# zhangxinsong-nlp/XFM

Hardware: AMD Instinct MI355X
Metric: image-text pairs/sec fwd+bwd, XFM-base 224px/30tok (higher is better)
Workload: dtype bf16; 1 GPU; Pretrain.py full multimodal step (ITC+ITM+MLM+MIM), XFM-base, synthetic 224px images + 30-token captions, random init; units_per_gpu=64, global_batch=64, dropout=True, ordered_reductions=True, grad_allreduce=False, parallelism=dp1, image_res=224

## Files before the change

### xfm_amd/csrc/gemm.hip

```cpp
#include "common.h"

enum { EPI_BF16 = 0, EPI_F32 = 1, EPI_GELU = 2, EPI_DGELU = 3, EPI_F32_ACC = 4 };

#define XFM_FENCE() asm volatile("" ::: "memory")
#define XFM_BAR()                    \
  do {                               \
    XFM_FENCE();                     \
    __builtin_amdgcn_s_barrier();    \
    XFM_FENCE();                     \
  } while (0)


struct GemmNT {
  const bf16* A; long lda;
  const bf16* B; long ldb;
  void* C; long ldc;
  const float* bias;
  bf16* aux; long ldaux;
  int M, N, K;
  int group_m;
  int k_splits;
  long split_stride;
#ifdef XFM_DIAG
  long long* dbg;
// ... 810 lines not shown

__device__ __forceinline__ int swz_t(int r) { return ((r & 3) | (((r >> 3) & 1) << 2)) << 1; }

__device__ __forceinline__ bf16x8 tr_read_pair(const char* tile, int row0, int col0, int lr) {
  const int r = row0 + (lr >> 2);
  const int col = col0 + 4 * (lr & 3);
  const int off0 = r * 256 + ((((col >> 3)) ^ swz_t(r)) << 4) + (col & 7) * 2;
  const int r2 = r + 4;
  const int off1 = r2 * 256 + ((((col >> 3)) ^ swz_t(r2)) << 4) + (col & 7) * 2;
  const s16x4 lo = __builtin_amdgcn_ds_read_tr16_b64_v4i16(LDS_PTR(s16x4, tile + off0));
  const s16x4 hi = __builtin_amdgcn_ds_read_tr16_b64_v4i16(LDS_PTR(s16x4, tile + off1));
  union { struct { s16x4 a, b; } s; bf16x8 v; } u;
  u.s.a = lo;
  u.s.b = hi;
  return u.v;
}

__global__ __launch_bounds__(256) void gemm_tn_kernel(GemmTN g) {
  constexpr int TILE = 64 * 256;
  extern __shared__ __attribute__((aligned(16))) char smem[];
  const int tid = threadIdx.x, lane = tid & 63, w = tid >> 6;
  const int wn = w >> 1, wk = w & 1;
  const int lr = lane & 15, lg = lane >> 4;
  const int tiles_k = (g.K + 127) / 128, tiles_n = (g.N + 127) / 128;
  const int per_split = tiles_k * tiles_n;
  const int wg = xcd_remap(blockIdx.x, gridDim.x);
  const int split = wg / per_split, t = wg % per_split;
  const int n0 = (t / tiles_k) * 128, k0 = (t % tiles_k) * 128;
  const int mbeg = split * g.m_per_split;
  int mend = mbeg + g.m_per_split;
  mend = mend < g.M ? mend : g.M;
  const int nsteps = (mend - mbeg + 63) / 64;

  const bool do_bias = g.dbias != nullptr && k0 == 0;
  float bsum[8] = {0.f, 0.f, 0.f, 0.f, 0.f, 0.f, 0.f, 0.f};
  u32x4 ry[4], rx[4];
  auto gload = [&](int step) {
    const int mb = mbeg + step * 64;
#pragma unroll
    for (int i = 0; i < 4; ++i) {
      const int q = i * 256 + tid, r = q >> 4, c = q & 15;
      const int m = mb + r;
      const bool okm = m < mend;
      const int nn = n0 + c * 8, kk = k0 + c * 8;
      ry[i] = u32x4{0, 0, 0, 0};
      rx[i] = u32x4{0, 0, 0, 0};
      if (okm && nn < g.N) {
        if (nn + 8 <= g.N) ry[i] = *reinterpret_cast<const u32x4*>(g.dY + (long)m * g.ldy + nn);
        else {
          union { bf16 h[8]; u32x4 v; } u; u.v = u32x4{0, 0, 0, 0};
          for (int e = 0; e < 8; ++e) if (nn + e < g.N) u.h[e] = g.dY[(long)m * g.ldy + nn + e];
          ry[i] = u.v;
        }
      }
      if (okm && kk < g.K) rx[i] = *reinterpret_cast<const u32x4*>(g.X + (long)m * g.ldx + kk);
    }
  };
  auto lstore = [&](int buf) {
    char* sY = smem + buf * 2 * TILE;
    char* sX = sY + TILE;
#pragma unroll
    for (int i = 0; i < 4; ++i) {
      const int q = i * 256 + tid, r = q >> 4, c = q & 15;
      const int off = r * 256 + ((c ^ swz_t(r)) << 4);
      *reinterpret_cast<u32x4*>(sY + off) = ry[i];
      *reinterpret_cast<u32x4*>(sX + off) = rx[i];
      if (do_bias) {
#pragma unroll
        for (int e = 0; e < 4; ++e) {
          bsum[2 * e] += __uint_as_float(ry[i][e] << 16);
          bsum[2 * e + 1] += __uint_as_float(ry[i][e] & 0xFFFF0000u);
        }
      }
    }
  };

  f32x4 acc[4][4];
#pragma unroll
  for (int i = 0; i < 4; ++i)
#pragma unroll
    for (int j = 0; j < 4; ++j) acc[i][j] = f32x4{0.f, 0.f, 0.f, 0.f};

  if (nsteps > 0) {
    gload(0);
    lstore(0);
  }
  __syncthreads();
  for (int s = 0; s < nsteps; ++s) {
    const int cur = s & 1;
    if (s + 1 < nsteps) gload(s + 1);
    const char* sY = smem + cur * 2 * TILE;
    const char* sX = sY + TILE;
#pragma unroll
    for (int ks = 0; ks < 2; ++ks) {
      bf16x8 af[4], bfr[4];
#pragma unroll
      for (int nt = 0; nt < 4; ++nt) af[nt] = tr_read_pair(sY, ks * 32 + 8 * lg, wn * 64 + nt * 16, lr);
#pragma unroll
      for (int kt = 0; kt < 4; ++kt) bfr[kt] = tr_read_pair(sX, ks * 32 + 8 * lg, wk * 64 + kt * 16, lr);
#pragma unroll
      for (int nt = 0; nt < 4; ++nt)
#pragma unroll
        for (int kt = 0; kt < 4; ++kt)
          acc[nt][kt] = __builtin_amdgcn_mfma_f32_16x16x32_bf16(af[nt], bfr[kt], acc[nt][kt], 0, 0, 0);
    }
    if (s + 1 < nsteps) lstore(cur ^ 1);
    __syncthreads();
  }

  if (do_bias) {
    float* red = reinterpret_cast<float*>(smem);
    __syncthreads();
#pragma unroll
    for (int e = 0; e < 8; ++e) red[(tid >> 4) * 128 + (tid & 15) * 8 + e] = bsum[e];
    __syncthreads();
    if (tid < 128 && n0 + tid < g.N) {
      float t2 = 0.f;
#pragma unroll
      for (int r = 0; r < 16; ++r) t2 += red[r * 128 + tid];
      atomicAdd(g.dbias + n0 + tid, t2);
    }
  }
  if (g.ws != nullptr) {
    f32x4* wsp = reinterpret_cast<f32x4*>(g.ws) + ((((long)split * per_split + t) * 4 + w) * 16) * 64 + lane;
#pragma unroll
    for (int nt = 0; nt < 4; ++nt)
#pragma unroll
      for (int kt = 0; kt < 4; ++kt) wsp[(nt * 4 + kt) * 64] = acc[nt][kt];
    return;
  }
#pragma unroll
  for (int nt = 0; nt < 4; ++nt)
#pragma unroll
    for (int kt = 0; kt < 4; ++kt) {
      const int k = k0 + wk * 64 + kt * 16 + lr;
#pragma unroll
      for (int rgi = 0; rgi < 4; ++rgi) {
        const int n = n0 + wn * 64 + nt * 16 + 4 * lg + rgi;
        if (n < g.N && k < g.K) {
          float* dst = g.dW + (long)n * g.ldw + k;
          if (g.direct) *dst += acc[nt][kt][rgi];
          else atomicAdd(dst, acc[nt][kt][rgi]);
        }
      }
    }
}


__device__ __attribute__((aligned(256))) static const uint32_t g_zero_row[64] = {0};

__global__ __launch_bounds__(256) void gemm_tn_ring_kernel(GemmTN g, TnBatch bt) {
  constexpr int IMG = 32 * 256, STG = 2 * IMG, NS = 4;
  extern __shared__ __attribute__((aligned(16))) char smem[];
  const int tid = threadIdx.x, lane = tid & 63, w = tid >> 6;
  const int wn = w >> 1, wk = w & 1;
  const int lr = lane & 15, lg = lane >> 4;
  const int tiles_k = g.K / 128, tiles_n = g.N / 128;
  const int per_split = tiles_k * tiles_n;
  int wg = xcd_remap(blockIdx.x, gridDim.x);
  if (bt.nb > 1) {
    const int bi = wg / bt.wg_per;
    wg -= bi * bt.wg_per;
    g.dY = bt.dY[bi];
    g.X = bt.X[bi];
    g.dW = bt.dW[bi];
    g.dbias = bt.dbias[bi];
    g.ws += (long)bi * bt.ws_stride;
  }
  const int split = wg / per_split, t = wg % per_split;
  const int n0 = (t / tiles_k) * 128, k0 = (t % tiles_k) * 128;
  const int mbeg = split * g.m_per_split;
  int mend = mbeg + g.m_per_split;
  mend = mend < g.M ? mend : g.M;
  const int nsteps = (mend - mbeg + 31) / 32;
  const bool do_bias = g.dbias != nullptr && k0 == 0 && wk == 0;

  const bf16* zrow = reinterpret_cast<const bf16*>(g_zero_row);
  int lrow[2], lcol[2];
#pragma unroll
  for (int i = 0; i < 2; ++i) {
    lrow[i] = 4 * (i * 4 + w) + (lane >> 4);
    lcol[i] = ((lane & 15) ^ swz_t(lrow[i])) * 8;
  }
  auto issue = [&](int s) {
    if (s >= nsteps) return;
    char* base = smem + (s & (NS - 1)) * STG;
#pragma unroll
    for (int i = 0; i < 2; ++i) {
      const int m = mbeg + s * 32 + lrow[i];
      const bool ok = m < mend;
      const bf16* sy = ok ? g.dY + (long)m * g.ldy + n0 + lcol[i] : zrow + lcol[i];
      const bf16* sx = ok ? g.X + (long)m * g.ldx + k0 + lcol[i] : zrow + lcol[i];
      const unsigned dy_lds = (unsigned)(uintptr_t)LDS_PTR(void, base) + (unsigned)__builtin_amdgcn_readfirstlane((i * 4 + w) * 1024);
      asm volatile("s_mov_b32 m0, %1\n\ts_nop 0\n\tglobal_load_lds_dwordx4 %0, off" ::"v"(sy), "s"(dy_lds) : "memory", "m0");
      asm volatile("s_mov_b32 m0, %1\n\ts_nop 0\n\tglobal_load_lds_dwordx4 %0, off" ::"v"(sx), "s"(dy_lds + (unsigned)IMG) : "memory", "m0");
    }
  };

  f32x4 acc[4][4];
#pragma unroll
  for (int i = 0; i < 4; ++i)
#pragma unroll
    for (int j = 0; j < 4; ++j) acc[i][j] = f32x4{0.f, 0.f, 0.f, 0.f};
  f32x4 bacc[4];
#pragma unroll
  for (int i = 0; i < 4; ++i) bacc[i] = f32x4{0.f, 0.f, 0.f, 0.f};
  bf16x8 ones;
#pragma unroll
  for (int i = 0; i < 8; ++i) ones[i] = f2bf(1.0f);

  issue(0);
  issue(1);
  issue(2);
  for (int s = 0; s < nsteps; ++s) {
    const int younger = nsteps - 1 - s < 2 ? nsteps - 1 - s : 2;
    if (younger == 2) asm volatile("s_waitcnt vmcnt(8)" ::: "memory");
    else if (younger == 1) asm volatile("s_waitcnt vmcnt(4)" ::: "memory");
    else asm volatile("s_waitcnt vmcnt(0)" ::: "memory");
    XFM_BAR();
    issue(s + 3);
    const char* sY = smem + (s & (NS - 1)) * STG;
    const char* sX = sY + IMG;
    bf16x8 af[4], bfr[4];
#pragma unroll
    for (int nt = 0; nt < 4; ++nt) af[nt] = tr_read_pair(sY, 8 * lg, wn * 64 + nt * 16, lr);
#pragma unroll
    for (int kt = 0; kt < 4; ++kt) bfr[kt] = tr_read_pair(sX, 8 * lg, wk * 64 + kt * 16, lr);
#pragma unroll
    for (int nt = 0; nt < 4; ++nt)
#pragma unroll
      for (int kt = 0; kt < 4; ++kt)
        acc[nt][kt] = __builtin_amdgcn_mfma_f32_16x16x32_bf16(af[nt], bfr[kt], acc[nt][kt], 0, 0, 0);
    if (do_bias) {
#pragma unroll
      for (int nt = 0; nt < 4; ++nt) bacc[nt] = __builtin_amdgcn_mfma_f32_16x16x32_bf16(af[nt], ones, bacc[nt], 0, 0, 0);
    }
  }

  if (do_bias && lr == 0) {
#pragma unroll
    for (int nt = 0; nt < 4; ++nt)
#pragma unroll
      for (int i = 0; i < 4; ++i) atomicAdd(g.dbias + n0 + wn * 64 + nt * 16 + 4 * lg + i, bacc[nt][i]);
  }
  if (g.ws != nullptr) {
    f32x4* wsp = reinterpret_cast<f32x4*>(g.ws) + ((((long)split * per_split + t) * 4 + w) * 16) * 64 + lane;
#pragma unroll
    for (int nt = 0; nt < 4; ++nt)
#pragma unroll
      for (int kt = 0; kt < 4; ++kt) wsp[(nt * 4 + kt) * 64] = acc[nt][kt];
    return;
  }
#pragma unroll
  for (int nt = 0; nt < 4; ++nt)
#pragma unroll
    for (int kt = 0; kt < 4; ++kt) {
      const int k = k0 + wk * 64 + kt * 16 + lr;
#pragma unroll
      for (int rgi = 0; rgi < 4; ++rgi) {
        const int n = n0 + wn * 64 + nt * 16 + 4 * lg + rgi;
        float* dst = g.dW + (long)n * g.ldw + k;
        if (g.direct) *dst += acc[nt][kt][rgi];
        else atomicAdd(dst, acc[nt][kt][rgi]);
      }
    }
}

__global__ __launch_bounds__(256) void tn_reduce128_kernel(const float* __restrict__ ws, float* __restrict__ dW, long ldw, int N, int K,
                                                           int tiles_k, int per_split, int splits, TnBatch bt) {
  if (bt.nb > 1) {
    ws += (long)blockIdx.y * bt.ws_stride;
    dW = bt.dW[blockIdx.y];
  }
  const long idx = (long)blockIdx.x * 256 + threadIdx.x;
  const int lane = (int)(idx & 63), q = (int)((idx >> 6) & 15), w = (int)((idx >> 10) & 3);
  const int t = (int)(idx >> 12);
  if (t >= per_split) return;
  const f32x4* p = reinterpret_cast<const f32x4*>(ws) + idx;
  const long stride = (long)per_split * 4 * 16 * 64;
  f32x4 sum = p[0];
  for (int sp = 1; sp < splits; ++sp) sum += p[sp * stride];
  const int n0 = (t / tiles_k) * 128, k0 = (t % tiles_k) * 128;
  const int wn = w >> 1, wk = w & 1, lr = lane & 15, lg = lane >> 4, nt = q >> 2, kt = q & 3;
  const int k = k0 + wk * 64 + kt * 16 + lr;
  const int n = n0 + wn * 64 + nt * 16 + 4 * lg;
  if (k >= K) return;
#pragma unroll
  for (int i = 0; i < 4; ++i)
    if (n + i < N) dW[(long)(n + i) * ldw + k] += sum[i];
}

struct Tn256Seg {
  const bf16* dY; const bf16* X;
  unsigned ldy, ldx;
  int n0, k0, mbeg, nk;
  bool do_bias;
  int rows;
};
__device__ __attribute__((aligned(16))) const unsigned tn_zero16[4] = {0u, 0u, 0u, 0u};

template <bool RAGGED>
__device__ __forceinline__ void tn256_mainloop(const Tn256Seg& sg, char* smem, f32x4 (&acc)[8][4], f32x4 (&bacc)[2]) {
  constexpr int UNIT = 64 * 256, BUF = 4 * UNIT;
  const int tid = threadIdx.x, lane = tid & 63, w = tid >> 6;
  const int wr = w >> 2, wc = w & 3;
  const int lr = lane & 15, lg = lane >> 4;
  const int n0 = sg.n0, k0 = sg.k0, mbeg = sg.mbeg, nk = sg.nk;
  const int total = 4 * nk;
  const bool do_bias = sg.do_bias;

  unsigned soff[4][2];
  int doff[4][2];
#pragma unroll
  for (int i = 0; i < 2; ++i) {
    const int b = i * 8 + w;
    const int r = 4 * b + (lane >> 4);
    const int c = ((lane & 15) ^ swz_t(r)) * 8;
    const unsigned rowy = (unsigned)(mbeg + r) * (unsigned)sg.ldy, rowx = (unsigned)(mbeg + r) * (unsigned)sg.ldx;
    soff[0][i] = rowy + n0 + (c >> 6) * 128 + (c & 63);
    soff[3][i] = rowy + n0 + (c >> 6) * 128 + 64 + (c & 63);
    soff[1][i] = rowx + k0 + (c >> 5) * 64 + (c & 31);
    soff[2][i] = rowx + k0 + (c >> 5) * 64 + 32 + (c & 31);
    doff[0][i] = 0 * UNIT + b * 1024;
    doff[1][i] = 1 * UNIT + b * 1024;
    doff[2][i] = 2 * UNIT + b * 1024;
    doff[3][i] = 3 * UNIT + b * 1024;
  }
  auto issue = [&](int s) {
    if (s >= total) return;
    const int kt = s >> 2, j = s & 3;
    char* base = smem + (kt & 1) * BUF;
    const bool isy = (j == 0 || j == 3);
    const bf16* src = (isy ? sg.dY : sg.X) + (size_t)kt * 64 * (size_t)(isy ? sg.ldy : sg.ldx);
#pragma unroll
    for (int i = 0; i < 2; ++i) {
      const unsigned so = j == 0 ? soff[0][i] : j == 1 ? soff[1][i] : j == 2 ? soff[2][i] : soff[3][i];
      const int dofs = j == 0 ? doff[0][i] : j == 1 ? doff[1][i] : j == 2 ? doff[2][i] : doff[3][i];
      const unsigned lds_addr = (unsigned)(uintptr_t)LDS_PTR(void, base) + (unsigned)__builtin_amdgcn_readfirstlane(dofs);
      const bf16* ptr = src + (size_t)so;
      if (RAGGED && kt * 64 + 4 * (i * 8 + w) + (lane >> 4) >= sg.rows) ptr = reinterpret_cast<const bf16*>(tn_zero16);
      asm volatile("s_mov_b32 m0, %1\n\ts_nop 0\n\tglobal_load_lds_dwordx4 %0, off" ::"v"(ptr), "s"(lds_addr) : "memory", "m0");
    }
  };

#pragma unroll
  for (int i = 0; i < 8; ++i)
#pragma unroll
    for (int j = 0; j < 4; ++j) acc[i][j] = f32x4{0.f, 0.f, 0.f, 0.f};
  bacc[0] = bacc[1] = f32x4{0.f, 0.f, 0.f, 0.f};
  bf16x8 ones;
#pragma unroll
  for (int i = 0; i < 8; ++i) ones[i] = f2bf(1.0f);

  const int lrow = 8 * lg + (lr >> 2);
  const int tsw = swz_t(lrow);
  int offa[4], offb[2];
#pragma unroll
  for (int f = 0; f < 4; ++f) {
    const int col = wr * 64 + f * 16 + 4 * (lr & 3);
    offa[f] = lrow * 256 + (((col >> 3) ^ tsw) << 4) + (col & 7) * 2;
  }
#pragma unroll
  for (int f = 0; f < 2; ++f) {
    const int col = wc * 32 + f * 16 + 4 * (lr & 3);
    offb[f] = lrow * 256 + (((col >> 3) ^ tsw) << 4) + (col & 7) * 2;
  }
  auto tr_pair = [&](const char* p) {
    const s16x4 lo = __builtin_amdgcn_ds_read_tr16_b64_v4i16(LDS_PTR(s16x4, p));
    const s16x4 hi = __builtin_amdgcn_ds_read_tr16_b64_v4i16(LDS_PTR(s16x4, p + 1024));
    union { struct { s16x4 a, b; } s; bf16x8 v; } u;
    u.s.a = lo;
    u.s.b = hi;
    return u.v;
  };
  bf16x8 xa[4][2], wb0[2][2], wb1[2][2];
  auto read_a = [&](const char* unit) {
#pragma unroll
    for (int f = 0; f < 4; ++f) {
      xa[f][0] = tr_pair(unit + offa[f]);
      xa[f][1] = tr_pair(unit + offa[f] + 8192);
    }
  };
  auto read_b = [&](const char* unit, bf16x8 (&wb)[2][2]) {
#pragma unroll
    for (int f = 0; f < 2; ++f) {
      wb[f][0] = tr_pair(unit + offb[f]);
      wb[f][1] = tr_pair(unit + offb[f] + 8192);
    }
  };
#define XFM_TQUAD(MH, NH, WB)                                                                                    \
  do {                                                                                                           \
    __builtin_amdgcn_s_setprio(1);                                                                               \
    _Pragma("unroll") for (int ks = 0; ks < 2; ++ks)                                                             \
    _Pragma("unroll") for (int m = 0; m < 4; ++m)                                                                \
    _Pragma("unroll") for (int n = 0; n < 2; ++n)                                                                \
      acc[MH * 4 + m][NH * 2 + n] =                                                                              \
          __builtin_amdgcn_mfma_f32_16x16x32_bf16(xa[m][ks], WB[n][ks], acc[MH * 4 + m][NH * 2 + n], 0, 0, 0);  \
    __builtin_amdgcn_s_setprio(0);                                                                               \
  } while (0)
#define XFM_TBIAS(H)                                                                                             \
  do {                                                                                                           \
    if (do_bias) {                                                                                               \
      _Pragma("unroll") for (int f = 0; f < 4; ++f)                                                              \
        if (f == wc) {                                                                                           \
          bacc[H] = __builtin_amdgcn_mfma_f32_16x16x32_bf16(xa[f][0], ones, bacc[H], 0, 0, 0);                  \
          bacc[H] = __builtin_amdgcn_mfma_f32_16x16x32_bf16(xa[f][1], ones, bacc[H], 0, 0, 0);                  \
        }                                                                                                        \
    }                                                                                                            \
  } while (0)

#pragma unroll
  for (int s = 0; s < 5; ++s) issue(s);
  wait_younger((total - 1 < 4 ? total - 1 : 4) - 1);
  XFM_BAR();
  if (wr == 1) XFM_BAR();

  for (int kt = 0; kt < nk; ++kt) {
    const char* buf = smem + (kt & 1) * BUF;
    const int ph = 4 * kt;
    int last;
    issue(ph + 5);
    read_a(buf + 0 * UNIT);
    read_b(buf + 1 * UNIT, wb0);
    last = ph + 5 < total ? ph + 5 : total - 1;
    wait_younger(last - (ph + 2));
    XFM_BAR();
    XFM_TQUAD(0, 0, wb0);
    XFM_TBIAS(0);
    XFM_BAR();
    issue(ph + 6);
    read_b(buf + 2 * UNIT, wb1);
    last = ph + 6 < total ? ph + 6 : total - 1;
    wait_younger(last - (ph + 3));
    XFM_BAR();
    XFM_TQUAD(0, 1, wb1);
    XFM_BAR();
    issue(ph + 7);
    read_a(buf + 3 * UNIT);
    XFM_BAR();
    XFM_TQUAD(1, 1, wb1);
    XFM_TBIAS(1);
    XFM_BAR();
    issue(ph + 8);
    last = ph + 8 < total ? ph + 8 : total - 1;
    wait_younger(last - (ph + 5) < 0 ? 0 : last - (ph + 5));
    XFM_BAR();
    XFM_TQUAD(1, 0, wb0);
    XFM_BAR();
  }
  if (wr == 0) XFM_BAR();
#undef XFM_TQUAD
#undef XFM_TBIAS

}

template <bool ATOMIC>
__device__ __forceinline__ void tn256_bias_out(float* dbias, int n0, const f32x4 (&bacc)[2]) {
  const int lane = threadIdx.x & 63, w = threadIdx.x >> 6, wr = w >> 2, wc = w & 3, lr = lane & 15, lg = lane >> 4;
  if (lr != 0) return;
#pragma unroll
  for (int h = 0; h < 2; ++h)
#pragma unroll
    for (int i = 0; i < 4; ++i) {
      float* d = dbias + n0 + wr * 128 + h * 64 + wc * 16 + 4 * lg + i;
      if (ATOMIC) atomicAdd(d, bacc[h][i]);
      else *d += bacc[h][i];
    }
}
__device__ __forceinline__ void tn256_bias_part(float* part, const f32x4 (&bacc)[2]) {
  const int lane = threadIdx.x & 63, w = threadIdx.x >> 6, wr = w >> 2, wc = w & 3, lr = lane & 15, lg = lane >> 4;
  if (lr != 0) return;
#pragma unroll
  for (int h = 0; h < 2; ++h) *reinterpret_cast<f32x4*>(part + wr * 128 + h * 64 + wc * 16 + 4 * lg) = bacc[h];
}
__device__ __forceinline__ void tn256_store_partial(float* ws, long slot, const f32x4 (&acc)[8][4]) {
  const int lane = threadIdx.x & 63, w = threadIdx.x >> 6;
  f32x4* wsp = reinterpret_cast<f32x4*>(ws) + ((slot * 8 + w) * 32) * 64 + lane;
#pragma unroll
  for (int nt = 0; nt < 8; ++nt)
#pragma unroll
    for (int kt = 0; kt < 4; ++kt) wsp[(nt * 4 + kt) * 64] = acc[nt][kt];
}
template <bool ATOMIC>
__device__ __forceinline__ void tn256_add_out(float* dW, long ldw, int n0, int k0, const f32x4 (&acc)[8][4]) {
  const int lane = threadIdx.x & 63, w = threadIdx.x >> 6, wr = w >> 2, wc = w & 3, lr = lane & 15, lg = lane >> 4;
#pragma unroll
  for (int nt = 0; nt < 8; ++nt)
#pragma unroll
    for (int kt = 0; kt < 4; ++kt) {
      const int k = k0 + wc * 64 + kt * 16 + lr;
#pragma unroll
      for (int rgi = 0; rgi < 4; ++rgi) {
        const int n = n0 + wr * 128 + nt * 16 + 4 * lg + rgi;
        if (ATOMIC) atomicAdd(dW + (long)n * ldw + k, acc[nt][kt][rgi]);
        else dW[(long)n * ldw + k] += acc[nt][kt][rgi];
      }
    }
}

__global__ __launch_bounds__(512) void gemm_tn_256_kernel(GemmTN g) {
  extern __shared__ __attribute__((aligned(16))) char smem[];
  const int tiles_k = g.K / 256, tiles_n = g.N / 256;
  const int per_split = tiles_k * tiles_n;
  const int wg = xcd_remap(blockIdx.x, gridDim.x);
  const int split = wg / per_split, t = wg % per_split;
  const int n0 = (t / tiles_k) * 256, k0 = (t % tiles_k) * 256;
  const int mbeg = split * g.m_per_split;
  int mend = mbeg + g.m_per_split;
  mend = mend < g.M ? mend : g.M;
  const Tn256Seg sg{g.dY, g.X, (unsigned)g.ldy, (unsigned)g.ldx, n0, k0, mbeg, (mend - mbeg) / 64, g.dbias != nullptr && k0 == 0, 0};
  f32x4 acc[8][4], bacc[2];
  tn256_mainloop<false>(sg, smem, acc, bacc);
  if (sg.do_bias) tn256_bias_out<true>(g.dbias, n0, bacc);
  if (g.ws != nullptr) {
    tn256_store_partial(g.ws, (long)split * per_split + t, acc);
    return;
  }
  tn256_add_out<true>(g.dW, g.ldw, n0, k0, acc);
}

#define TN_GROUP_MAX 48
struct TnGroupProb {
  const bf16* dY; const bf16* X;
  float* dW; float* dbias;
  unsigned ldy, ldx;
  long ldw;
  int tiles_k;
  int tile_end;
};
struct TnGroup {
  int nprob, nk;
  int M;
  int total_tiles, full_tiles;
  int sk_wgs;
  long sk_iters;
  float* ws;
  float* ws_bias;
  TnGroupProb p[TN_GROUP_MAX];
};
__host__ __device__ __forceinline__ long tn_sk_bound(long R, int nk, int sk_wgs, int i) {
  long raw = (long)i * R / sk_wgs;
  const int rem = (int)(raw % nk);
  if (rem < 4) raw -= rem;
  else if (nk - rem < 4) raw += nk - rem;
  return raw;
}

__global__ __launch_bounds__(512) void gemm_tn_group_kernel(TnGroup G) {
  extern __shared__ __attribute__((aligned(16))) char smem[];
  const int wg = xcd_remap(blockIdx.x, gridDim.x), nwg = gridDim.x;
  int dp_t = wg;
  long sk_pos = 0, sk_end = 0;
  if (wg < G.sk_wgs) {
    sk_pos = tn_sk_bound(G.sk_iters, G.nk, G.sk_wgs, wg);
    sk_end = tn_sk_bound(G.sk_iters, G.nk, G.sk_wgs, wg + 1);
  }
  const long sk_a = sk_pos;
  bool first = true;
  for (;;) {
    int tile, it0, it1;
    long slot = -1;
    if (dp_t < G.full_tiles) {
      tile = dp_t;
      dp_t += nwg;
      it0 = 0;
      it1 = G.nk;
    } else if (sk_pos < sk_end) {
      const int rt = (int)(sk_pos / G.nk);
      const long t_end = (long)(rt + 1) * G.nk;
      it0 = (int)(sk_pos - (long)rt * G.nk);
      it1 = (int)((sk_end < t_end ? sk_end : t_end) - (long)rt * G.nk);
      tile = G.full_tiles + rt;
      if (it0 != 0 || it1 != G.nk) slot = 2l * wg + (sk_pos == sk_a ? 0 : 1);
      sk_pos = (long)rt * G.nk + it1;
    } else {
      break;
    }
    if (!first) __syncthreads();
    first = false;
    int pi = 0;
    while (pi + 1 < G.nprob && tile >= G.p[pi].tile_end) ++pi;
    const TnGroupProb& P = G.p[pi];
    const int tl = tile - (pi > 0 ? G.p[pi - 1].tile_end : 0);
    const int n0 = (tl / P.tiles_k) * 256, k0 = (tl % P.tiles_k) * 256;
    const Tn256Seg sg{P.dY, P.X, P.ldy, P.ldx, n0, k0, it0 * 64, it1 - it0, P.dbias != nullptr && k0 == 0, G.M - it0 * 64};
    f32x4 acc[8][4], bacc[2];
    tn256_mainloop<true>(sg, smem, acc, bacc);
    if (slot >= 0) {
      if (sg.do_bias) tn256_bias_part(G.ws_bias + slot * 256, bacc);
      tn256_store_partial(G.ws, slot, acc);
    } else {
      if (sg.do_bias) tn256_bias_out<false>(P.dbias, n0, bacc);
      tn256_add_out<false>(P.dW, P.ldw, n0, k0, acc);
    }
  }
}

__global__ __launch_bounds__(256) void tn_group_fixup_kernel(TnGroup G) {
  const int rt = blockIdx.y;
  const int idx = blockIdx.x * 256 + threadIdx.x;
  const long R = G.sk_iters;
  const long a = (long)rt * G.nk, b = a + G.nk;
  int i0 = (int)(a * G.sk_wgs / R);
  i0 = i0 < G.sk_wgs - 1 ? i0 : G.sk_wgs - 1;
  while (i0 > 0 && tn_sk_bound(R, G.nk, G.sk_wgs, i0) > a) --i0;
  while (i0 + 1 < G.sk_wgs && tn_sk_bound(R, G.nk, G.sk_wgs, i0 + 1) <= a) ++i0;
  int i1 = i0;
  while (i1 + 1 < G.sk_wgs && tn_sk_bound(R, G.nk, G.sk_wgs, i1 + 1) < b) ++i1;
  if (i0 == i1) return;
  const f32x4* ws = reinterpret_cast<const f32x4*>(G.ws);
  f32x4 sum = f32x4{0.f, 0.f, 0.f, 0.f};
  for (int i = i0; i <= i1; ++i) {
    const long slot = 2l * i + (tn_sk_bound(R, G.nk, G.sk_wgs, i) >= a ? 0 : 1);
    sum += ws[slot * (8 * 32 * 64) + idx];
  }
  const int tile = G.full_tiles + rt;
  int pi = 0;
  while (pi + 1 < G.nprob && tile >= G.p[pi].tile_end) ++pi;
  const TnGroupProb& P = G.p[pi];
  const int tl = tile - (pi > 0 ? G.p[pi - 1].tile_end : 0);
  const int n0 = (tl / P.tiles_k) * 256, k0 = (tl % P.tiles_k) * 256;
  const int lane = idx & 63, q = (idx >> 6) & 31, w = idx >> 11;
  const int wr = w >> 2, wc = w & 3, lr = lane & 15, lg = lane >> 4, nt = q >> 2, kt = q & 3;
  const int k = k0 + wc * 64 + kt * 16 + lr;
  const int n = n0 + wr * 128 + nt * 16 + 4 * lg;
#pragma unroll
  for (int i = 0; i < 4; ++i) P.dW[(long)(n + i) * P.ldw + k] += sum[i];
  if (blockIdx.x == 0 && P.dbias != nullptr && k0 == 0) {
    float b = 0.f;
    for (int i = i0; i <= i1; ++i) {
      const long slot = 2l * i + (tn_sk_bound(R, G.nk, G.sk_wgs, i) >= a ? 0 : 1);
      b += G.ws_bias[slot * 256 + threadIdx.x];
    }
    P.dbias[n0 + threadIdx.x] += b;
  }
}

__global__ __launch_bounds__(256) void tn_reduce_kernel(const float* __restrict__ ws, float* __restrict__ dW, long ldw, int tiles_k,
                                                        int per_split, int splits) {
  const long idx = (long)blockIdx.x * 256 + threadIdx.x;
  const int lane = (int)(idx & 63), q = (int)((idx >> 6) & 31), w = (int)((idx >> 11) & 7);
  const int t = (int)(idx >> 14);
  if (t >= per_split) return;
  const f32x4* p = reinterpret_cast<const f32x4*>(ws) + idx;
  const long stride = (long)per_split * 8 * 32 * 64;
  f32x4 sum = p[0];
  for (int sp = 1; sp < splits; ++sp) {
    const f32x4 v = p[sp * stride];
    sum += v;
  }
  const int n0 = (t / tiles_k) * 256, k0 = (t % tiles_k) * 256;
  const int wr = w >> 2, wc = w & 3, lr = lane & 15, lg = lane >> 4, nt = q >> 2, kt = q & 3;
  const int k = k0 + wc * 64 + kt * 16 + lr;
  const int n = n0 + wr * 128 + nt * 16 + 4 * lg;
#pragma unroll
  for (int i = 0; i < 4; ++i) dW[(long)(n + i) * ldw + k] += sum[i];
}

static int tn256_plan(int M, int N, int K, int& splits, int& mps) {
  const int t256 = (N / 256) * (K / 256);
  splits = 256 / t256;
  const int steps = M / 64;
  if (splits > steps / 8) splits = steps / 8;
  if (splits < 1) splits = 1;
  mps = cdiv(steps, splits) * 64;
  splits = cdiv(M, mps);
  return t256;
}

static bool tn256_eligible(long ldy, long ldx, int M, int N, int K) {
  return M % 64 == 0 && N % 256 == 0 && K % 256 == 0 && N >= 256 && K >= 256 &&
         (unsigned long)M * (unsigned long)(ldy > ldx ? ldy : ldx) < (1ul << 32);
}

#define TN_WS_MIN_BYTES (16l << 20)

static int tn128_plan(int M, int N, int K, int splits_hint, int& splits, int& mps) {
  const int tiles = cdiv(N, 128) * cdiv(K, 128);
  splits = splits_hint < 0 ? 0 : splits_hint;
  if (splits <= 0) {
    splits = (432 + tiles / 2) / tiles;
    int max_splits = M / 480;
    if (max_splits < 2 && M >= 640) max_splits = 2;
    if (splits > max_splits) splits = max_splits;
    if (splits < 1) splits = 1;
  }
  mps = cdiv(cdiv(M, splits), 64) * 64;
  splits = cdiv(M, mps);
  return tiles;
}

static int tn256_body_rows(int M, int N, int K) {
  const int M0 = M - M % 64;
  static const int min_rows = xfm_env_int("XFM_TN256_RAGGED_MIN", 8192);
  if (M % 64 == 0 || M0 < min_rows || N % 256 != 0 || K % 256 != 0) return 0;
  int splits, mps;
  return tn256_plan(M0, N, K, splits, mps) >= 18 ? M0 : 0;
}

long xfm_gemm_tn_workspace_impl(int M, int N, int K) {
  if (M <= 0 || N <= 0 || K <= 0) return 0;
  int splits, mps;
  if (const int M0 = tn256_body_rows(M, N, K)) return xfm_gemm_tn_workspace_impl(M0, N, K);
  if (tn256_eligible(N, K, M, N, K)) {
    const int t256 = tn256_plan(M, N, K, splits, mps);
    if (t256 >= 18 && M >= 4096) return (long)splits * N * K * 4;
  }
  const int tiles = tn128_plan(M, N, K, 0, splits, mps);
  const long need = (long)splits * tiles * 128 * 128 * 4;
  return (splits > 1 && need >= TN_WS_MIN_BYTES) ? need : 0;
}

int xfm_gemm_tn_impl(const void* dY, long ldy, const void* X, long ldx, float* dW, long ldw, float* dbias, int M, int N, int K,
                     int splits_hint, float* workspace, long workspace_bytes, hipStream_t st) {
  XFM_REQUIRE(M > 0 && N > 0 && K > 0, "gemm_tn: empty problem M=%d N=%d K=%d", M, N, K);
  XFM_REQUIRE(K % 8 == 0 && ldx % 8 == 0 && ldy % 8 == 0, "gemm_tn: K=%d ldx=%ld ldy=%ld must be multiples of 8", K, ldx, ldy);
  XFM_REQUIRE(((uintptr_t)dY % 16) == 0 && ((uintptr_t)X % 16) == 0, "gemm_tn: operands must be 16-byte aligned");
  if (splits_hint == 0) {
    if (const int M0 = tn256_body_rows(M, N, K)) {
      if (tn256_eligible(ldy, ldx, M0, N, K) && workspace != nullptr && workspace_bytes >= xfm_gemm_tn_workspace_impl(M0, N, K)) {
        int rc = xfm_gemm_tn_impl(dY, ldy, X, ldx, dW, ldw, dbias, M0, N, K, 0, workspace, workspace_bytes, st);
        if (rc != XFM_OK) return rc;
        return xfm_gemm_tn_impl((const bf16*)dY + (long)M0 * ldy, ldy, (const bf16*)X + (long)M0 * ldx, ldx, dW, ldw, dbias, M - M0, N, K, 1,
                                workspace, workspace_bytes, st);
      }
    }
  }
  if (tn256_eligible(ldy, ldx, M, N, K) && splits_hint != -4) {
    int splits, mps;
    const int t256 = tn256_plan(M, N, K, splits, mps);
    const long need = (long)splits * N * K * 4;
    const bool have_ws = workspace != nullptr && workspace_bytes >= need;
    const bool want = splits_hint == -3 || (splits_hint == 0 && t256 >= 18 && M >= 4096 && have_ws);
    if (want) {
      GemmTN g{(const bf16*)dY, ldy, (const bf16*)X, ldx, dW, ldw, dbias, M, N, K, mps, have_ws ? workspace : nullptr, 0};
      static bool attr256 = false;
      const size_t smem256 = 2 * 4 * 64 * 256;
      if (!attr256) {
        (void)hipFuncSetAttribute(reinterpret_cast<const void*>(gemm_tn_256_kernel), hipFuncAttributeMaxDynamicSharedMemorySize,
                                  (int)smem256);
        attr256 = true;
      }
      hipLaunchKernelGGL(gemm_tn_256_kernel, dim3(t256 * splits), dim3(512), smem256, st, g);
      int rc = xfm_check_launch("gemm_tn_256");
      if (rc != XFM_OK || !have_ws) return rc;
      const long quads = (long)t256 * 8 * 32 * 64;
      hipLaunchKernelGGL(tn_reduce_kernel, dim3((unsigned)cdiv(quads, 256)), dim3(256), 0, st, workspace, dW, ldw, K / 256, t256, splits);
      return xfm_check_launch("gemm_tn_reduce");
    }
  }
  int splits, mps;
  const int tiles = tn128_plan(M, N, K, splits_hint, splits, mps);
  const long need = (long)splits * tiles * 128 * 128 * 4;
  const bool use_ws = splits > 1 && workspace != nullptr && workspace_bytes >= need && (need >= TN_WS_MIN_BYTES || splits_hint > 0);
  GemmTN g{(const bf16*)dY, ldy, (const bf16*)X, ldx, dW, ldw, dbias, M, N, K, mps, use_ws ? workspace : nullptr, splits == 1 ? 1 : 0};
  static bool attr_set = false;
// ... 293 lines not shown
```

Before: 1717 pairs/s.

## Interleave LDS transpose reads with MFMAs in TN256 weight-grad mainloop

```diff
diff --git a/xfm_amd/csrc/gemm.hip b/xfm_amd/csrc/gemm.hip
--- a/xfm_amd/csrc/gemm.hip
+++ b/xfm_amd/csrc/gemm.hip
@@ -1136,7 +1136,7 @@
 template <bool RAGGED>
 __device__ __forceinline__ void tn256_mainloop(const Tn256Seg& sg, char* smem, f32x4 (&acc)[8][4], f32x4 (&bacc)[2]) {
   constexpr int UNIT = 64 * 256, BUF = 4 * UNIT;
-  const int tid = threadIdx.x, lane = tid & 63, w = tid >> 6;
+  const int tid = threadIdx.x, lane = tid & 63, w = __builtin_amdgcn_readfirstlane(tid >> 6);
   const int wr = w >> 2, wc = w & 3;
   const int lr = lane & 15, lg = lane >> 4;
   const int n0 = sg.n0, k0 = sg.k0, mbeg = sg.mbeg, nk = sg.nk;
@@ -1177,6 +1177,14 @@
     }
   };
 
+  auto stage = [&](int q) {
+    if (q >= total) return;
+    issue(q + 5);
+    if ((q & 3) == 2) return;
+    const int last = q + 5 < total ? q + 5 : total - 1;
+    wait_younger(last - (q + 2) < 0 ? 0 : last - (q + 2));
+  };
+
 #pragma unroll
   for (int i = 0; i < 8; ++i)
 #pragma unroll
@@ -1199,14 +1207,15 @@
     const int col = wc * 32 + f * 16 + 4 * (lr & 3);
     offb[f] = lrow * 256 + (((col >> 3) ^ tsw) << 4) + (col & 7) * 2;
   }
-  auto tr_pair = [&](const char* p) {
-    const s16x4 lo = __builtin_amdgcn_ds_read_tr16_b64_v4i16(LDS_PTR(s16x4, p));
-    const s16x4 hi = __builtin_amdgcn_ds_read_tr16_b64_v4i16(LDS_PTR(s16x4, p + 1024));
+  auto tr_lo = [&](const char* p) { return __builtin_amdgcn_ds_read_tr16_b64_v4i16(LDS_PTR(s16x4, p)); };
+  auto tr_hi = [&](const char* p) { return __builtin_amdgcn_ds_read_tr16_b64_v4i16(LDS_PTR(s16x4, p + 1024)); };
+  auto tr_join = [&](s16x4 lo, s16x4 hi) {
     union { struct { s16x4 a, b; } s; bf16x8 v; } u;
     u.s.a = lo;
     u.s.b = hi;
     return u.v;
   };
+  auto tr_pair = [&](const char* p) { return tr_join(tr_lo(p), tr_hi(p)); };
   bf16x8 xa[4][2], wb0[2][2], wb1[2][2];
   auto read_a = [&](const char* unit) {
 #pragma unroll
@@ -1222,15 +1231,62 @@
       wb[f][1] = tr_pair(unit + offb[f] + 8192);
     }
   };
-#define XFM_TQUAD(MH, NH, WB)                                                                                    \
-  do {                                                                                                           \
-    __builtin_amdgcn_s_setprio(1);                                                                               \
-    _Pragma("unroll") for (int ks = 0; ks < 2; ++ks)                                                             \
-    _Pragma("unroll") for (int m = 0; m < 4; ++m)                                                                \
-    _Pragma("unroll") for (int n = 0; n < 2; ++n)                                                                \
-      acc[MH * 4 + m][NH * 2 + n] =                                                                              \
-          __builtin_amdgcn_mfma_f32_16x16x32_bf16(xa[m][ks], WB[n][ks], acc[MH * 4 + m][NH * 2 + n], 0, 0, 0);  \
-    __builtin_amdgcn_s_setprio(0);                                                                               \
+#define XFM_TMFMA(MH, NH, WB, KS, M, N)                                                                           \
+  acc[MH * 4 + M][NH * 2 + N] =                                                                                   \
+      __builtin_amdgcn_mfma_f32_16x16x32_bf16(xa[M][KS], WB[N][KS], acc[MH * 4 + M][NH * 2 + N], 0, 0, 0)
+#define XFM_THALF(MH, NH, WB, KS)                                                                                 \
+  do {                                                                                                            \
+    _Pragma("unroll") for (int m = 0; m < 4; ++m) {                                                               \
+      XFM_TMFMA(MH, NH, WB, KS, m, 0);                                                                            \
+      XFM_TMFMA(MH, NH, WB, KS, m, 1);                                                                            \
+    }                                                                                                             \
+  } while (0)
+#define XFM_THALF_RDA(MH, NH, WB, KS, UNITP)                                                                      \
+  do {                                                                                                            \
+    _Pragma("unroll") for (int m = 0; m < 4; ++m) {                                                               \
+      XFM_TMFMA(MH, NH, WB, KS, m, 0);                                                                            \
+      const s16x4 lo_ = tr_lo((UNITP) + offa[m]);                                                                 \
+      XFM_TMFMA(MH, NH, WB, KS, m, 1);                                                                            \
+      const s16x4 hi_ = tr_hi((UNITP) + offa[m]);                                                                 \
+      xa[m][0] = tr_join(lo_, hi_);                                                                               \
+    }                                                                                                             \
+    XFM_TPIN(8, 1);                                                                                               \
+  } while (0)
+#define XFM_TRDA1(UNITP)                                                                                          \
+  do {                                                                                                            \
+    _Pragma("unroll") for (int f = 0; f < 4; ++f) xa[f][1] = tr_join(tr_lo((UNITP) + offa[f] + 8192), tr_hi((UNITP) + offa[f] + 8192)); \
+  } while (0)
+#define XFM_THALF_RDB(MH, NH, WB, KS, DST, UNITP)                                                                 \
+  do {                                                                                                            \
+    _Pragma("unroll") for (int m = 0; m < 4; ++m) {                                                               \
+      XFM_TMFMA(MH, NH, WB, KS, m, 0);                                                                            \
+      const s16x4 lo_ = tr_lo((UNITP) + offb[m & 1] + (m >> 1) * 8192);                                           \
+      XFM_TMFMA(MH, NH, WB, KS, m, 1);                                                                            \
+      const s16x4 hi_ = tr_hi((UNITP) + offb[m & 1] + (m >> 1) * 8192);                                           \
+      DST[m & 1][m >> 1] = tr_join(lo_, hi_);                                                                     \
+    }                                                                                                             \
+    XFM_TPIN(8, 1);                                                                                               \
+  } while (0)
+#define XFM_TQUAD_RDB(MH, NH, WB, DST, UNITP)                                                                     \
+  do {                                                                                                            \
+    _Pragma("unroll") for (int ks = 0; ks < 2; ++ks)                                                              \
+    _Pragma("unroll") for (int f = 0; f < 2; ++f) {                                                               \
+      XFM_TMFMA(MH, NH, WB, ks, 2 * f, 0);                                                                        \
+      XFM_TMFMA(MH, NH, WB, ks, 2 * f, 1);                                                                        \
+      const s16x4 lo_ = tr_lo((UNITP) + offb[f] + ks * 8192);                                                     \
+      XFM_TMFMA(MH, NH, WB, ks, 2 * f + 1, 0);                                                                    \
+      XFM_TMFMA(MH, NH, WB, ks, 2 * f + 1, 1);                                                                    \
+      const s16x4 hi_ = tr_hi((UNITP) + offb[f] + ks * 8192);                                                     \
+      DST[f][ks] = tr_join(lo_, hi_);                                                                             \
+    }                                                                                                             \
+    XFM_TPIN(8, 2);                                                                                               \
+  } while (0)
+#define XFM_TPIN(N, PER)                                                                                          \
+  do {                                                                                                            \
+    _Pragma("unroll") for (int i_ = 0; i_ < N; ++i_) {                                                            \
+      __builtin_amdgcn_sched_group_barrier(0x008, PER, 0);                                                        \
+      __builtin_amdgcn_sched_group_barrier(0x100, 1, 0);                                                          \
+    }                                                                                                             \
   } while (0)
 #define XFM_TBIAS(H)                                                                                             \
   do {                                                                                                           \
@@ -1242,50 +1298,85 @@
         }                                                                                                        \
     }                                                                                                            \
   } while (0)
+#define XFM_TNEXT(Q)                                                                                             \
+  do {                                                                                                           \
+    XFM_BAR();                                                                                                   \
+    if (wr == 0) stage(Q);        \
+    else stage((Q) + 1);                                                                                         \
+  } while (0)
+#define XFM_TTILE(KT, BX, BY)                                                                                    \
+  do {                                                                                                           \
+    const char* buf = smem + ((KT) & 1) * BUF;                                                                   \
+    const char* nbuf = smem + (((KT) + 1) & 1) * BUF;                                                            \
+    const int ph = 4 * (KT);                                                                                     \
+                                                                                \
+    XFM_BAR();                                                                                                   \
+    __builtin_amdgcn_s_setprio(1);                                                                               \
+    XFM_TQUAD_RDB(0, 0, BX, BY, buf + 2 * UNIT);                                                                 \
+    XFM_TBIAS(0);                                                                                                \
+    __builtin_amdgcn_s_setprio(0);                                                                               \
+    XFM_TNEXT(ph + 1);                                                                                     \
+                          \
+    XFM_BAR();                                                                                                   \
+    __builtin_amdgcn_s_setprio(1);                                                                               \
+    XFM_THALF(0, 1, BY, 0);                                                                                      \
+    __builtin_amdgcn_sched_barrier(0);                                                                           \
+    XFM_THALF_RDA(0, 1, BY, 1, buf + 3 * UNIT);                                                                  \
+    __builtin_amdgcn_sched_barrier(0);                                                                           \
+    __builtin_amdgcn_s_setprio(0);                                                                               \
+    XFM_TRDA1(buf + 3 * UNIT);                                                                                   \
+    XFM_TNEXT(ph + 2);                                                                                    \
+                                                         \
+    XFM_BAR();                                                                                                   \
+    __builtin_amdgcn_s_setprio(1);                                                                               \
+    XFM_THALF(1, 1, BY, 0);                                                                                      \
+    XFM_THALF(1, 1, BY, 1);                                                                                      \
+    XFM_TBIAS(1);                                                                                                \
+    __builtin_amdgcn_s_setprio(0);                                                                               \
+    XFM_TNEXT(ph + 3);                                                                                     \
+                              \
+    XFM_BAR();                                                                                                   \
+    __builtin_amdgcn_s_setprio(1);                                                                               \
+    XFM_THALF_RDB(1, 0, BX, 0, BY, nbuf + 1 * UNIT);                                                             \
+    __builtin_amdgcn_sched_barrier(0);                                                                           \
+    XFM_THALF_RDA(1, 0, BX, 1, nbuf + 0 * UNIT);                                                                 \
+    __builtin_amdgcn_sched_barrier(0);                                                                           \
+    __builtin_amdgcn_s_setprio(0);                                                                               \
+    XFM_TRDA1(nbuf + 0 * UNIT);                                                                                  \
+    XFM_TNEXT(ph + 4);                                                                                     \
+  } while (0)
 
 #pragma unroll
   for (int s = 0; s < 5; ++s) issue(s);
   wait_younger((total - 1 < 4 ? total - 1 : 4) - 1);
   XFM_BAR();
-  if (wr == 1) XFM_BAR();
+  read_a(smem + 0 * UNIT);
+  read_b(smem + 1 * UNIT, wb0);
+  stage(0);
+  if (wr == 1) {
+    stage(1);
+    XFM_BAR();
+  }
 
   for (int kt = 0; kt < nk; ++kt) {
-    const char* buf = smem + (kt & 1) * BUF;
-    const int ph = 4 * kt;
-    int last;
-    issue(ph + 5);
-    read_a(buf + 0 * UNIT);
-    read_b(buf + 1 * UNIT, wb0);
-    last = ph + 5 < total ? ph + 5 : total - 1;
-    wait_younger(last - (ph + 2));
-    XFM_BAR();
-    XFM_TQUAD(0, 0, wb0);
-    XFM_TBIAS(0);
-    XFM_BAR();
-    issue(ph + 6);
-    read_b(buf + 2 * UNIT, wb1);
-    last = ph + 6 < total ? ph + 6 : total - 1;
-    wait_younger(last - (ph + 3));
-    XFM_BAR();
-    XFM_TQUAD(0, 1, wb1);
-    XFM_BAR();
-    issue(ph + 7);
-    read_a(buf + 3 * UNIT);
-    XFM_BAR();
-    XFM_TQUAD(1, 1, wb1);
-    XFM_TBIAS(1);
-    XFM_BAR();
-    issue(ph + 8);
-    last = ph + 8 < total ? ph + 8 : total - 1;
-    wait_younger(last - (ph + 5) < 0 ? 0 : last - (ph + 5));
-    XFM_BAR();
-    XFM_TQUAD(1, 0, wb0);
-    XFM_BAR();
+    XFM_TTILE(kt, wb0, wb1);
+#pragma unroll
+    for (int f = 0; f < 2; ++f) {
+      wb0[f][0] = wb1[f][0];
+      wb0[f][1] = wb1[f][1];
+    }
   }
   if (wr == 0) XFM_BAR();
-#undef XFM_TQUAD
+#undef XFM_TMFMA
+#undef XFM_THALF
+#undef XFM_THALF_RDA
+#undef XFM_TRDA1
+#undef XFM_THALF_RDB
+#undef XFM_TQUAD_RDB
+#undef XFM_TPIN
 #undef XFM_TBIAS
-
+#undef XFM_TNEXT
+#undef XFM_TTILE
 }
 
 template <bool ATOMIC>
```

After: 1699 pairs/s, median of 2. No clear change (-1.0%).
